# NCAR/SPERR

Measured on AMD Instinct MI355X. Metric: compress+decompress GB/s/GPU on 256^3 fp32 chunks @ BPP=2.0; bitstream-exact vs ref, higher is better.
Workload: dtype f64; 1 GPU; synthetic 1024^3 fp32 turbulence per GPU, 256^3 chunks, BPP=2.0, step = compress + decompress, volume and container resident in HBM; chunks_per_gpu=64, parallelism=chunks farmed over 1 GPU(s), no collective

## Files before the change

sperr_amd/csrc/engine.hip:

```cpp
#include <algorithm>
#include <array>
#include <chrono>
#include <cstdlib>
#include <cstring>
#include <atomic>
#include <deque>
#include <map>
#include <memory>
#include <condition_variable>
#include <mutex>
#include <numeric>
#include <thread>
#include <string>
#include <vector>

#include "../../include/sperr_hip.h"
#include "engine_internal.h"
#include "host_container.hpp"
#include "speck_dec.h"
#include "speck_enc.h"
#include "speck_tree_host.hpp"
#include "outlier.h"
#include "xform.h"

// ... 1094 lines not shown
  e.pixCntStride = (size_t)kMaxPlanes * 2 * P.nPixTiles;
  TAKE(e.pixCnt, uint32_t, e.pixCntStride * B);
  TAKE(e.pixOff, uint32_t, e.pixCntStride * B);
  e.streamStride = streamWords;
  TAKE(e.stream, uint64_t, streamWords * B);
#undef TAKE
  return true;
}

size_t enc_bytes_for(const ShapePlan& P, uint32_t B, uint64_t raw_budget, bool alias = true)
{
  Arena probe;
  probe.base = reinterpret_cast<char*>(uintptr_t(4096));
  probe.cap = ~size_t(0) / 2;
  EncBatchBufs tmp;
  carve_enc(probe, P, std::max<uint32_t>(B, 1), raw_budget, tmp, alias);
  return probe.used;
}
size_t enc_bytes_per_chunk(const ShapePlan& P, uint64_t raw_budget, bool alias = true)
{
  return enc_bytes_for(P, 1, raw_budget, alias);
}

int reset_enc_pass(hipStream_t st, const EncBatchBufs& bb, uint32_t B)
{
  const EncBuffers& e = bb.eb;
  HIP_CHECK(hipMemsetAsync(e.bplane, 0xff, e.pixStride * B, st));
  HIP_CHECK(hipMemsetAsync(e.M, 0xff, e.nodeStride * B, st));
  HIP_CHECK(hipMemsetAsync(e.mask, 0, std::max<size_t>(e.maskStride, 1) * B * sizeof(uint64_t), st));
  HIP_CHECK(hipMemsetAsync(e.stream, 0, e.streamStride * B * sizeof(uint64_t), st));
  return 0;
}

bool fuse_xy(const ShapePlan& P)
{
  if (P.fwd.size() < 2 || P.fwd[0].axis != 0 || P.fwd[1].axis != 1)
    return false;
  for (int a = 0; a < 3; a++)
    if (P.fwd[0].region[a] != P.dims[a] || P.fwd[1].region[a] != P.dims[a])
      return false;
  return lift_xy_applicable(P.dims);
}

bool fuse_xyz(const ShapePlan& P)
{
  if (!fuse_xy(P) || P.fwd.size() < 3 || P.fwd[2].axis != 2)
    return false;
  for (int a = 0; a < 3; a++)
    if (P.fwd[2].region[a] != P.dims[a])
      return false;
  return lift_xyz_applicable(P.dims);
}

int pass_fuse(const ShapePlan& P, size_t k, uint32_t inner[3])
{
  const LiftPass& ps = P.fwd[k];
  inner[0] = inner[1] = inner[2] = 0;
  for (size_t j = k + 1; j < P.fwd.size(); j++)
    for (int a = 0; a < 3; a++)
      inner[a] = std::max(inner[a], P.fwd[j].region[a]);
  bool nested = k + 1 >= P.fwd.size();
  for (size_t j = k + 1; j < P.fwd.size(); j++)
    nested = nested || (P.fwd[j].region[0] == inner[0] && P.fwd[j].region[1] == inner[1] &&
                        P.fwd[j].region[2] == inner[2]);
  if (!nested)
    return -1;
  bool covers = true;
  for (int a = 0; a < 3; a++)
    covers = covers && inner[a] >= ps.region[a];
  return covers ? 0 : 1;
}

bool plan_fusable(const ShapePlan& P)
{
  if (P.fwd.empty())
    return false;
  uint32_t inner[3];
  for (size_t k = 0; k < P.fwd.size(); k++)
    if (pass_fuse(P, k, inner) < 0)
      return false;
  if (fuse_xy(P) && (pass_fuse(P, 0, inner) != 0 || pass_fuse(P, 1, inner) != 0))
    return false;
  return true;
}

template <typename T>
int float_stages(hipStream_t ss, const ShapePlan& P, EncBatchBufs& bb, uint32_t nb, const uint32_t cd[3],
                 const T* d_src, VolDesc vd, bool orgAligned, bool wantRange)
{
  EncBuffers& e = bb.eb;
  const bool fuse = !P.fwd.empty();
  const int io = std::is_same<T, float>::value ? 1 : 2;
  if (launch_condition<T>(ss, d_src, vd, bb.geom, nb, cd, P.nstrides, bb.strideMean, bb.strideMeanStride,
                          bb.vals, bb.valsStride, e.cst, !fuse, wantRange, orgAligned))
    return -1;
  size_t k0 = 0;
  const bool fuseMax = plan_fusable(P);
  if (fuse_xyz(P)) {
    LiftFuse lf;
    if (fuseMax && pass_fuse(P, 2, lf.inner) > 0)
      lf.mode = 1;
    if (launch_lift_xyz(ss, true, bb.vals, bb.valsStride, nb, cd, e.cst, io, const_cast<T*>(d_src), vd,
                        bb.geom, &lf))
      return -1;
    k0 = 3;
  }
  else if (fuse_xy(P)) {
    if (launch_lift_xy(ss, true, bb.vals, bb.valsStride, nb, cd, e.cst, io, const_cast<T*>(d_src), vd,
                       bb.geom))
      return -1;
    k0 = 2;
  }
  for (size_t k = k0; k < P.fwd.size(); k++) {
    const LiftPass& ps = P.fwd[k];
    LiftFuse lf;
    if (fuseMax && pass_fuse(P, k, lf.inner) > 0)
      lf.mode = 1;
    if (launch_lift(ss, true, bb.vals, bb.valsStride, nb, cd, ps.axis, ps.region, e.cst, k == 0 ? io : 0,
                    const_cast<T*>(d_src), vd, bb.geom, &lf))
      return -1;
  }
  return 0;
}

int unalias_coder(hipStream_t ss, Engine& E, const ShapePlan& P, EncBatchBufs& bb, uint32_t nb)
{
  HIP_CHECK(hipStreamSynchronize(ss));
  if (E.wideScratch.ensure(bb.coderBytes + 4096))
    return -1;
  Arena W;
  W.base = static_cast<char*>(E.wideScratch.p);
  W.cap = E.wideScratch.n;
  if (!carve_enc_coder(W, nullptr, P, nb, bb.eb))
    return -1;
  bb.aliased = false;
  return 0;
}

template <typename T>
int wide_retry_prepare(hipStream_t ss, Engine& E, const ShapePlan& P, EncBatchBufs& bb, uint32_t nb,
                       const uint32_t cd[3], const T* d_src, VolDesc vd, bool orgAligned, bool wantRange)
{
  if (unalias_coder(ss, E, P, bb, nb))
    return -1;
  g_dbg_counter[0]++;
  return float_stages<T>(ss, P, bb, nb, cd, d_src, vd, orgAligned, wantRange);
}

int psnr_q_search(hipStream_t st, const ShapePlan& P, EncBatchBufs& bb, uint32_t nb, double psnr,
                  std::vector<CoderState>& hc, std::vector<CoderState>& got)
{
  EncBuffers& e = bb.eb;
  hc.assign(nb, CoderState{});
  HIP_CHECK(hipMemcpyAsync(hc.data(), e.cst, nb * sizeof(CoderState), hipMemcpyDeviceToHost, st));
  HIP_CHECK(hipStreamSynchronize(st));
  std::vector<double> tmse(nb, 0.0);
  bool any = false;
  for (uint32_t i = 0; i < nb; i++) {
// ... 1748 lines not shown
    double* boxVals = nullptr;
    size_t boxStride = 0;
    ChunkGeom* d_bricks = nullptr;
    if (fbrick) {
      for (size_t k = 3; k < P.fwd.size(); k++)
        for (int a = 0; a < 3; a++)
          bbox[a] = std::max(bbox[a], P.fwd[k].region[a]);
      boxStride = round_up((size_t)bbox[0] * bbox[1] * bbox[2], 64);
      const size_t geomOff = round_up((size_t)nb * boxStride * 8, 256);
      if (E.decBox[q].ensure(geomOff + (size_t)nb * sizeof(ChunkGeom) + 256))
        return -1;
      boxVals = static_cast<double*>(E.decBox[q].p);
      d_bricks = reinterpret_cast<ChunkGeom*>(static_cast<char*>(E.decBox[q].p) + geomOff);
      S.bricks.resize(nb);
      for (uint32_t i = 0; i < nb; i++) {
        S.bricks[i].org[0] = (uint32_t)((size_t)i * bb.valsStride);
        S.bricks[i].org[1] = S.bricks[i].org[2] = 0;
      }
      HIP_CHECK(hipMemcpyAsync(d_bricks, S.bricks.data(), nb * sizeof(ChunkGeom), hipMemcpyHostToDevice, ss));
    }
    const size_t perLevel = slice ? 2 : 3;
    auto sub_volume = [&](size_t k) -> int {
      if (!mr || !mr->nlev)
        return 0;
      const size_t h = mr->nlev - (k / perLevel + 1);
      const auto& r = mr->cres[h];
      const uint32_t blocks = capped_blocks((r[0] * r[1] * r[2] + kThreads - 1) / kThreads, nb);
      LAUNCH_K(k_sub_volume, dim3(blocks, nb), dim3(kThreads), 0, ss, bb.vals, bb.valsStride, d.cst, bb.geom,
               cd[0], cd[1], cd[0], cd[1], cd[2], r[0], r[1], r[2], mr->grid[0], mr->grid[1], mr->d_level[h]);
      return 0;
    };
    auto dequant_fuse = [&](size_t k, LiftFuse& lf) {
      if (b.fuseDq && pass_fuse(P, k, lf.inner) > 0) {
        lf.mode = 2;
        lf.coef = bb.coef32;
        lf.coefStride = d.coefStride;
        lf.sign = d.sign;
        lf.signStride = d.signStride;
        lf.sigNew = d.sigNew;
        lf.sigOld = d.sigOld;
        lf.maskStride = d.maskPixStride;
        lf.dst = d.st;
        lf.coefSigned = d.refPlanes ? 1 : 0;
      }
      if (b.compactElems) {
        lf.bufx = b.cbox[0];
        lf.bufy = b.cbox[1];
      }
      if (fbrick) {
        lf.bufx = bbox[0];
        lf.bufy = bbox[1];
      }
    };
    for (size_t k = P.fwd.size(); k-- > ((fxyz || fbrick) ? 3u : fxy ? 2u : 0u);) {
      const LiftPass& ps = P.fwd[k];
      if (k % perLevel == perLevel - 1 && sub_volume(k))
        return -1;
      LiftFuse lf;
      dequant_fuse(k, lf);
      const bool last = k == 0 && !S.outliers;
      if (launch_lift(ss, false, fbrick ? boxVals : bb.vals, fbrick ? boxStride : bb.valsStride, nb, cd, ps.axis,
                      ps.region, d.cst, last ? io : 0, d_dst, vd, bb.geom, &lf, last ? bb.crop : nullptr))
        return -1;
    }
    if (fbrick) {
      LiftFuse lf;
      dequant_fuse(2, lf);
      lf.noMean = 1;
      const VolDesc brickVol{{cd[0], cd[1], cd[2]}};
      if (launch_lift_xyz(ss, false, boxVals, boxStride, nb, cd, d.cst, 2, bb.vals, brickVol, d_bricks, &lf))
        return -1;
    }
    if (fxyz) {
      if (sub_volume(2))
        return -1;
      LiftFuse lf;
      dequant_fuse(2, lf);
      if (launch_lift_xyz(ss, false, bb.vals, bb.valsStride, nb, cd, d.cst, io, d_dst, vd, bb.geom, &lf, bb.crop))
        return -1;
    }
    if (fxy && slice && sub_volume(1))
      return -1;
    if (fxy && launch_lift_xy(ss, false, bb.vals, bb.valsStride, nb, cd, d.cst, io, d_dst, vd, bb.geom, bb.crop))
      return -1;
    if (S.outliers) {
      HIP_CHECK(hipStreamWaitEvent(ss, E.evOutl[q], 0));
      if (launch_outlier_apply(ss, S.ob, d.cst, bb.vals, bb.valsStride))
        return -1;
      HIP_CHECK(hipMemcpyAsync(S.hoc.data(), S.ob.oc, nb * sizeof(OutlierChunk), hipMemcpyDeviceToHost, ss));
      HIP_CHECK(hipStreamSynchronize(ss));
      for (auto& o : S.hoc)
        if (o.error) {
          fprintf(stderr, "[sperr_hip] outlier decoder failed (code %u)\n", o.error);
          return -1;
        }
    }
    if ((P.fwd.empty() || S.outliers) &&
        launch_scatter<T>(ss, d_dst, vd, bb.geom, nb, cd, bb.vals, bb.valsStride, d.cst, bb.crop))
      return -1;
    return 0;
  }
  int collect_states(const Batch& b)
  {
    for (uint32_t q = 0; q < b.nsub; q++) {
      SubHost& S = (*b.subs)[q];
      if (S.nb == 0)
        continue;
      hipStream_t ss = b.nsub > 1 ? E.sub[q] : st;
      if (S.bb.db.lisStamps && q == 0) {
        g_lis_stamps_host.assign(64, 0);
        const uint32_t sc = getenv("SPERR_HIP_STAMP_CHUNK")
                                ? std::min<uint32_t>(S.nb - 1, (uint32_t)atoi(getenv("SPERR_HIP_STAMP_CHUNK")))
                                : 0u;
        HIP_CHECK(hipMemcpyAsync(g_lis_stamps_host.data(), S.bb.db.lisStamps + (size_t)sc * 64, 64 * 8,
                                 hipMemcpyDeviceToHost, ss));
// ... 1348 lines not shown
```

sperr_amd/csrc/xform.h:

```cpp
#ifndef SPERR_AMD_XFORM_H
#define SPERR_AMD_XFORM_H

#include <string.h>

#include "common.h"

namespace sperrhip {

struct LiftConsts {
  double alpha, beta, gamma, delta, eps, inv_eps;
};
LiftConsts lift_consts();

template <typename T>
int launch_condition(hipStream_t stream, const T* vol, VolDesc vd, const ChunkGeom* geom,
                     uint32_t nchunks, const uint32_t cdims[3], uint32_t nstrides,
                     double* strideMean, size_t strideMeanStride, double* vals,
                     size_t valsStride, CoderState* st, bool gather, bool want_range = false,
                     bool org_x_aligned = false);

template <typename T>
int launch_scatter(hipStream_t stream, T* vol, VolDesc vd, const ChunkGeom* geom,
                   uint32_t nchunks, const uint32_t cdims[3], const double* vals,
                   size_t valsStride, const CoderState* st, const CropGeom* crop = nullptr);

struct DecState;
struct LiftFuse {
  int mode = 0;
  uint32_t inner[3] = {0, 0, 0};
  const uint32_t* coef = nullptr;
  size_t coefStride = 0;
  const uint64_t* sign = nullptr;
  size_t signStride = 0;
  const uint64_t* sigNew = nullptr;
  const uint64_t* sigOld = nullptr;
  size_t maskStride = 0;
  const DecState* dst = nullptr;
  int coefSigned = 0;
  int noMean = 0;
  uint32_t bufx = 0, bufy = 0;
};

int launch_lift(hipStream_t stream, bool forward, double* vals, size_t valsStride,
                uint32_t nchunks, const uint32_t cdims[3], int axis, const uint32_t region[3],
                CoderState* st, int io = 0, void* volume = nullptr, VolDesc vd = VolDesc{},
                const ChunkGeom* geom = nullptr, const LiftFuse* fuse = nullptr,
                const CropGeom* crop = nullptr);

bool lift_xy_applicable(const uint32_t cdims[3]);
int launch_lift_xy(hipStream_t stream, bool forward, double* vals, size_t valsStride,
                   uint32_t nchunks, const uint32_t cdims[3], const CoderState* st, int io,
                   void* volume, VolDesc vd, const ChunkGeom* geom, const CropGeom* crop = nullptr);

bool lift_xyz_applicable(const uint32_t cdims[3]);
int launch_lift_xyz(hipStream_t stream, bool forward, double* vals, size_t valsStride, uint32_t nchunks,
                    const uint32_t cdims[3], CoderState* st, int io, void* volume, VolDesc vd,
                    const ChunkGeom* geom, const LiftFuse* fuse, const CropGeom* crop = nullptr);

int launch_maxabs_q(hipStream_t stream, const double* vals, size_t valsStride, uint32_t nchunks,
                    uint32_t n, CoderState* st, bool have_max = false);
int launch_make_q_wide(hipStream_t stream, uint32_t nchunks, CoderState* st);
int launch_mark_wide(hipStream_t stream, uint32_t nchunks, CoderState* st);

int launch_mse(hipStream_t stream, const double* vals, size_t valsStride, uint32_t nchunks,
               uint32_t n, double* partial, size_t partialStride, CoderState* st);

__host__ __device__ inline unsigned long long order_key(double v)
{
  unsigned long long b;
  memcpy(&b, &v, 8);
  return (b >> 63) ? ~b : (b | 0x8000000000000000ull);
}
__host__ __device__ inline double order_key_value(unsigned long long k)
{
  const unsigned long long b = (k >> 63) ? (k & 0x7fffffffffffffffull) : ~k;
  double v;
  memcpy(&v, &b, 8);
  return v;
}

int launch_quantize(hipStream_t stream, bool wide, const double* vals, size_t valsStride,
                    uint32_t nchunks, uint32_t n, void* coef, size_t coefStride, uint64_t* sign,
                    size_t signStride, int8_t* msb, size_t msbStride, const CoderState* st);

int launch_inv_quantize(hipStream_t stream, bool wide, const void* coef, size_t coefStride,
                        const uint64_t* sign, size_t signStride, uint32_t nchunks, uint32_t n,
                        double* vals, size_t valsStride, const CoderState* st,
                        const uint64_t* sigNew = nullptr, const uint64_t* sigOld = nullptr,
                        size_t maskStride = 0, const DecState* dst = nullptr);

}

#endif
```

sperr_amd/csrc/xform.hip:

```cpp
#include <type_traits>

#include "xform.h"
#include "speck_dec.h"

namespace sperrhip {


constexpr int kSumStrides = 64, kSumSeg = 64;


template <typename T>
__global__ void __launch_bounds__(kThreads)
k_stride_sums(const T* __restrict__ vol, VolDesc vd, const ChunkGeom* geom, uint32_t cx,
              uint32_t cy, uint32_t cz, uint32_t nstrides, uint32_t ssz, double* strideMean,
              size_t strideMeanStride, CoderState* st, int want_range)
{
  __shared__ double tile[kSumStrides][kSumSeg + 1];
  __shared__ uint32_t sh_differs;
  double vmax = -INFINITY, vnegmax = -INFINITY;
  const uint32_t c = blockIdx.y;
  const uint32_t s0 = blockIdx.x * kSumStrides;
  const ChunkGeom g = geom[c];
  const size_t vx = vd.dims[0], vy = vd.dims[1];
  const T first = vol[((size_t)g.org[2] * vy + g.org[1]) * vx + g.org[0]];
// ... 736 lines not shown
                                           uint32_t jhi, uint32_t tid, const LiftConsts& K)
{
  const uint32_t nseg = (cx + kSeg - 1) / kSeg;
  const uint32_t ntask = (jhi - jlo) * nseg;
#pragma unroll 1
  for (uint32_t t = tid; t < ntask; t += NT) {
    const uint32_t rows = jhi - jlo, sg = t / rows, rb = jlo + (t - sg * rows);
    const double* row = src + (size_t)rb * RS + sg * kSeg;
    double r[16];
#pragma unroll
    for (int k = 0; k < 16; k++)
      r[k] = row[k];
    lift16<FORWARD>(r, K);
    double* out = dst + (size_t)rb * RS + 4 + sg * kSeg;
#pragma unroll
    for (int k = 0; k < kSeg; k++)
      if (sg * kSeg + k < cx)
        out[k] = r[4 + k];
  }
}

template <bool FORWARD, bool APRON, int NT>
__device__ __forceinline__ void xyz_lift_y(const double* src, double* dst, uint32_t RS, uint32_t cx, uint32_t nt,
                                           uint32_t tid, const LiftConsts& K)
{
  const uint32_t nq = (nt + kSeg - 1) / kSeg;
  const uint32_t ntask = nq * cx;
#pragma unroll 1
  for (uint32_t t = tid; t < ntask; t += NT) {
    const uint32_t q = t / cx, x = t - q * cx;
    const double* top = src + (size_t)(q * kSeg) * RS + 4 + x;
    double r[16];
#pragma unroll
    for (int k = 0; k < 16; k++)
      r[k] = top[(size_t)k * RS];
    lift16<FORWARD>(r, K);
#pragma unroll
    for (int k = 0; k < kSeg; k++) {
      if (q * kSeg + k < nt) {
        double* row = dst + (size_t)(4 + q * kSeg + k) * RS;
        if (APRON)
          xyz_put(row, x, cx, r[4 + k]);
        else
          row[4 + x] = r[4 + k];
      }
    }
  }
}

template <int IO>
__global__ void __launch_bounds__(kXYZThreadsF) __attribute__((amdgpu_waves_per_eu(kXYZThreadsF / 256, kXYZThreadsF / 256)))
k_lift_xyz_fwd(double* vals, size_t valsStride, uint32_t cx, uint32_t cy, uint32_t cz, LiftConsts K,
               CoderState* st, const void* volume, VolDesc vd, const ChunkGeom* geom, int wantMax,
               uint32_t in0, uint32_t in1, uint32_t in2, uint32_t nseg)
{
  static_assert(IO == 1 || IO == 2, "float or double volume");
  using VT = typename std::conditional<IO == 1, float, double>::type;
  const uint32_t c = blockIdx.y;
  if (st[c].is_const != 0)
    return;
  const uint32_t tid = threadIdx.x;
  const uint32_t seg = blockIdx.x % nseg, npairsAll = (cz + 1) / 2;
  const uint32_t mA = seg == 0 ? 0u : (uint32_t)((uint64_t)npairsAll * seg / nseg);
  const uint32_t mB = seg + 1 == nseg ? npairsAll : (uint32_t)((uint64_t)npairsAll * (seg + 1) / nseg);
  const uint32_t zFirst = mA >= 6 ? 2 * (mA - 6) : 0u;
  const uint32_t zEnd = seg + 1 == nseg ? cz : 2 * mB - 1;
  const uint32_t y0 = (blockIdx.x / nseg) * kXYZRows;
  const uint32_t nt = min((uint32_t)kXYZRows, cy - y0);
  const uint32_t RS = xyz_row_stride(cx);
  double* sm = reinterpret_cast<double*>(dyn_smem);
  const uint32_t bufN = (uint32_t)kXYZStaged * RS;
  const uint32_t xe = cx - cx / 2, ye = cy - cy / 2, ze = cz - cz / 2;
  const VT* vol = reinterpret_cast<const VT*>(volume);
  const size_t vsy = vd.dims[0], vsz = (size_t)vd.dims[0] * vd.dims[1];
  const VT* volc = vol + ((size_t)geom[c].org[2] * vsz + (size_t)geom[c].org[1] * vsy + geom[c].org[0]);
  double* buf = vals + c * valsStride;
  const size_t sliceN = (size_t)cx * cy;
  const double mean = st[c].mean;

  const uint32_t nstage = (uint32_t)kXYZStaged * cx;
  uint32_t pk[kXYZStageF];
#pragma unroll
  for (int k = 0; k < kXYZStageF; k++) {
    const uint32_t q = tid + (uint32_t)k * kXYZThreadsF;
    const uint32_t j = q / cx, x = q - j * cx;
    pk[k] = (j << 27) | (reflect_index((int)y0 - kXYHalo + (int)j, (int)cy) << 12) | x;
  }
  const uint32_t npos = nt * cx;
  uint32_t srow[kXYZPosF], ooff[kXYZPosF];
  uint32_t outerMask = 0;
#pragma unroll
  for (int k = 0; k < kXYZPosF; k++) {
    const uint32_t q = tid + (uint32_t)k * kXYZThreadsF;
    const uint32_t row = q / cx, col = q - row * cx, y = y0 + row;
    srow[k] = ((row + kXYHalo) << 16) | col;
    const uint32_t drow = (y & 1) ? ye + (y >> 1) : (y >> 1), dcol = (col & 1) ? xe + (col >> 1) : (col >> 1);
    ooff[k] = drow * cx + dcol;
    if (!(dcol < in0 && drow < in1))
      outerMask |= 1u << k;
  }
  double sxe[kXYZPosF], sxo[kXYZPosF], d1p[kXYZPosF], e1p[kXYZPosF], d2p[kXYZPosF];
#pragma unroll
  for (int k = 0; k < kXYZPosF; k++)
    sxe[k] = sxo[k] = d1p[k] = e1p[k] = d2p[k] = 0.0;
  double vmax = 0.0;
  auto emit = [&](int k, uint32_t zp, double v) {
    buf[(size_t)zp * sliceN + ooff[k]] = v;
    if (wantMax && (((outerMask >> k) & 1u) || zp >= in2))
      vmax = fmax(vmax, fabs(v));
  };

  VT pre[kXYZStageF];
  auto issue = [&](uint32_t z) {
    const VT* src = volc + (size_t)z * vsz;
#pragma unroll
    for (int k = 0; k < kXYZStageF; k++)
      pre[k] = (tid + (uint32_t)k * kXYZThreadsF) < nstage
                   ? src[(size_t)((pk[k] >> 12) & 0x7fffu) * vsy + (pk[k] & 0xfffu)] : (VT)0;
  };
  issue(zFirst);
  for (uint32_t z = zFirst; z < zEnd; z++) {
    uint32_t RSv = RS, tidv = tid;
    asm volatile("" : "+s"(RSv), "+v"(tidv));
#pragma unroll
    for (int k = 0; k < kXYZStageF; k++)
      asm volatile("" : "+v"(pk[k]));
#pragma unroll
    for (int k = 0; k < kXYZPosF; k++)
      asm volatile("" : "+v"(srow[k]), "+v"(ooff[k]));
    double* A = sm + ((z & 1) ? bufN : 0u);
    double* B = sm + ((z & 1) ? 0u : bufN);
#pragma unroll
    for (int k = 0; k < kXYZStageF; k++)
      if ((tid + (uint32_t)k * kXYZThreadsF) < nstage)
        xyz_put(A + (pk[k] >> 27) * RSv, pk[k] & 0xfffu, cx, (double)pre[k] - mean);
    if (z + 1 < zEnd)
      issue(z + 1);
    XYZ_LDS_BARRIER();
    xyz_lift_x<true, kXYZThreadsF>(A, B, RSv, cx, 0, kXYZStaged, tidv, K);
    XYZ_LDS_BARRIER();
    xyz_lift_y<true, false, kXYZThreadsF>(B, A, RSv, cx, nt, tidv, K);
    XYZ_LDS_BARRIER();
    const uint32_t m = z >> 1;
    if (z & 1) {
#pragma unroll
      for (int k = 0; k < kXYZPosF; k++)
        if ((tid + (uint32_t)k * kXYZThreadsF) < npos)
          sxo[k] = A[(srow[k] >> 16) * RSv + 4 + (srow[k] & 0xffffu)];
    }
    else {
#pragma unroll
      for (int k = 0; k < kXYZPosF; k++) {
        if ((tid + (uint32_t)k * kXYZThreadsF) >= npos)
          continue;
        const double v = A[(srow[k] >> 16) * RSv + 4 + (srow[k] & 0xffffu)];
        if (m >= 1) {
          const double d1n = fma(K.alpha, sxe[k] + v, sxo[k]);
          const double e1n = fma(K.beta, (m == 1 ? d1n : d1p[k]) + d1n, sxe[k]);
          if (m >= 2) {
            const double d2n = fma(K.gamma, e1p[k] + e1n, d1p[k]);
            const double e2 = K.eps * fma(K.delta, (m == 2 ? d2n : d2p[k]) + d2n, e1p[k]);
// ... 29 lines not shown
    }
    else {
      const uint32_t M = cz / 2;
      const double e1M = fma(K.beta, d1p[k] + d1p[k], sxe[k]);
      const double d2a = fma(K.gamma, e1p[k] + e1M, d1p[k]);
      const double e2a = K.eps * fma(K.delta, d2p[k] + d2a, e1p[k]);
      const double e2L = K.eps * fma(K.delta, d2a + d2a, e1M);
      emit(k, M - 1, e2a);
      emit(k, ze + M - 1, (-K.inv_eps) * d2a);
      emit(k, M, e2L);
    }
  }
  if (wantMax) {
    for (int d = 32; d > 0; d >>= 1)
      vmax = fmax(vmax, __shfl_xor(vmax, d, 64));
    if ((tid & 63) == 0 && vmax > 0.0)
      atomicMax(reinterpret_cast<unsigned long long*>(&st[c].maxabs),
                (unsigned long long)__double_as_longlong(vmax));
  }
}

template <int IO, bool SG, bool kCrop = false>
__global__ void __launch_bounds__(kXYZThreadsI) __attribute__((amdgpu_waves_per_eu(kXYZThreadsI / 256, kXYZThreadsI / 256)))
k_lift_xyz_inv(const double* vals, size_t valsStride, uint32_t cx, uint32_t cy, uint32_t cz, LiftConsts K,
               const CoderState* st, void* volume, VolDesc vd, const GeomOf<kCrop>* geom, LiftFuse F, uint32_t nseg)
{
  static_assert(IO == 1 || IO == 2, "float or double volume");
  using VT = typename std::conditional<IO == 1, float, double>::type;
  const uint32_t c = blockIdx.y;
  const uint32_t tid = threadIdx.x;
  const uint32_t seg = blockIdx.x % nseg, npairsAll = cz / 2;
  const uint32_t mA = seg == 0 ? 0u : (uint32_t)((uint64_t)npairsAll * seg / nseg);
  const uint32_t mB = seg + 1 == nseg ? npairsAll : (uint32_t)((uint64_t)npairsAll * (seg + 1) / nseg);
  const uint32_t mFirst = mA >= 6 ? mA - 6 : 0u;
  const uint32_t y0 = (blockIdx.x / nseg) * kXYZRows;
  const uint32_t nt = min((uint32_t)kXYZRows, cy - y0);
  const uint32_t RS = xyz_row_stride(cx);
  double* sm = reinterpret_cast<double*>(dyn_smem);
  const uint32_t bufN = (uint32_t)kXYZStaged * RS;
  const uint32_t xe = cx - cx / 2, ye = cy - cy / 2, ze = cz - cz / 2;
  VT* vol = reinterpret_cast<VT*>(volume);
  const size_t vsy = vd.dims[0], vsz = (size_t)vd.dims[0] * vd.dims[1];
  VT* volc = vol;
  CropGeom cg{};
  uint32_t wy0 = 0, wy1 = 0;
  if constexpr (kCrop) {
    cg = geom[c];
    wy0 = max(y0, cg.lo[1]) - y0;
    wy1 = min(y0 + nt, cg.hi[1]);
    if (y0 + wy0 >= wy1)
      return;
    wy1 -= y0;
  }
  else
    volc = vol + ((size_t)geom[c].org[2] * vsz + (size_t)geom[c].org[1] * vsy + geom[c].org[0]);
  auto crop_row = [&](uint32_t z, uint32_t r) -> VT* { return vol + crop_addr(cg, vd, cg.lo[0], y0 + r, z); };
  (void)crop_row;
  const double* buf = vals + c * valsStride;
  const size_t sliceN = (size_t)cx * cy;
  const uint32_t bufx = F.bufx ? F.bufx : cx;
  const size_t bufSlice = (size_t)bufx * (F.bufy ? F.bufy : cy);
  const double mean = st[c].mean;
  const uint32_t lane = tid & 63u, wave = tid >> 6, nwaves = kXYZThreadsI / 64;

  if (st[c].is_const != 0) {
    if constexpr (kCrop) {
      const uint32_t w = cg.hi[0] - cg.lo[0], nr = wy1 - wy0;
      for (uint32_t z = cg.lo[2] + seg; z < cg.hi[2]; z += nseg)
        for (uint32_t k = tid; k < nr * w; k += kXYZThreadsI)
          crop_row(z, wy0 + k / w)[k % w] = (VT)mean;
    }
    else
    for (uint32_t z = seg; z < cz; z += nseg)
      for (uint32_t k = tid; k < nt * cx; k += kXYZThreadsI)
        volc[(size_t)z * vsz + (size_t)(y0 + k / cx) * vsy + k % cx] = (VT)mean;
    return;
  }

  const uint32_t npos = (uint32_t)kXYZStaged * cx;
  uint32_t pk[kXYZPosI];
  uint32_t innerMask = 0;
#pragma unroll
  for (int k = 0; k < kXYZPosI; k++) {
    const uint32_t q = tid + (uint32_t)k * kXYZThreadsI;
    const uint32_t j = q / cx, x = q - j * cx, y = reflect_index((int)y0 - kXYHalo + (int)j, (int)cy);
    const uint32_t drow = (y & 1) ? ye + (y >> 1) : (y >> 1), dcol = (x & 1) ? xe + (x >> 1) : (x >> 1);
    pk[k] = (j << 27) | (y << 12) | x;
    if (dcol < F.inner[0] && drow < F.inner[1])
      innerMask |= 1u << k;
  }
  const bool dequant = F.mode == 2 && !st[c].wide;
  const double fq = dequant ? st[c].q : 0.0;
  const uint32_t* coef = F.coef + c * F.coefStride;
  const uint64_t* sign = F.sign + c * F.signStride;
  const bool haveMasks = dequant && F.sigNew != nullptr && F.dst != nullptr;
  const uint64_t* mNew = haveMasks ? F.sigNew + c * F.maskStride : sign;
  const uint64_t* mOld = haveMasks ? F.sigOld + c * F.maskStride : sign;
  const uint32_t lastPl = haveMasks ? (uint32_t)F.dst[c].lastPlane : 0u;
  const uint32_t initNew = haveMasks ? (1u << lastPl) + (1u << lastPl) - (1u << lastPl) / 2 - 1 : 0u;
  const uint32_t initOld = (haveMasks && lastPl < 31) ? (2u << lastPl) + (2u << lastPl) - (2u << lastPl) / 2 - 1 : 0u;
  const int scheme = (SG && dequant && F.dst) ? coef_scheme(F.dst[c]) : 0;
  const bool two = scheme == 2;
  auto sg_value = [&](uint32_t sv) -> double {
    double d = fq * (double)coef_scheme_mag(sv, two);
    return __hiloint2double(__double2hiint(d) ^ (int)(sv & 0x80000000u), __double2loint(d));
  };
  auto fetch = [&](int k, uint32_t zp) -> double {
    const uint32_t y = (pk[k] >> 12) & 0x7fffu, x = pk[k] & 0xfffu;
    const uint32_t drow = (y & 1) ? ye + (y >> 1) : (y >> 1), dcol = (x & 1) ? xe + (x >> 1) : (x >> 1);
    const size_t idx = (size_t)zp * sliceN + drow * cx + dcol;
    const bool inBox = ((innerMask >> k) & 1u) && zp < F.inner[2];
    if (!dequant && !inBox && F.bufx)
      return 0.0;
    if (dequant && !inBox) {
      if (SG && scheme)
        return sg_value(coef[idx]);
      uint32_t v = coef[idx];
      const uint32_t sh = (uint32_t)(idx & 63);
      const uint64_t sgw = sign[idx >> 6], mnw = mNew[idx >> 6], mow = mOld[idx >> 6];
      const uint32_t fill = ((mnw >> sh) & 1ull) ? initNew : (((mow >> sh) & 1ull) ? initOld : 0u);
      v = v ? v : fill;
      return fq * (double)v * (((sgw >> sh) & 1ull) ? 1.0 : -1.0);
    }
    return buf[(size_t)zp * bufSlice + drow * bufx + dcol];
  };
  uint32_t flip = 0;
  auto stage = [&](int k, double v) {
    uint32_t p = pk[k];
    asm volatile("" : "+v"(p));
    (sm + (flip ? bufN : 0u))[(p >> 27) * RS + 4 + (p & 0xfffu)] = v;
  };
  auto stage_all = [&](const double (&v)[kXYZPosI]) {
#pragma unroll
    for (int k = 0; k < kXYZPosI; k++)
      if ((tid + (uint32_t)k * kXYZThreadsI) < npos)
        stage(k, v[k]);
  };
  auto store_rows = [&](uint32_t z, uint32_t which) {
    const double* X = sm + (which ? bufN : 0u);
    if constexpr (kCrop) {
      if (z - cg.lo[2] >= cg.hi[2] - cg.lo[2])
        return;
      for (uint32_t r = wy0 + wave; r < wy1; r += nwaves) {
        VT* dstrow = crop_row(z, r);
        const double* srow = X + (size_t)(kXYHalo + r) * RS + 4;
        for (uint32_t x = cg.lo[0] + lane; x < cg.hi[0]; x += 64)
          dstrow[x - cg.lo[0]] = (VT)(F.noMean ? srow[x] : srow[x] + mean);
      }
      return;
    }
    for (uint32_t r = wave; r < nt; r += nwaves) {
      VT* dstrow = volc + (size_t)z * vsz + (size_t)(y0 + r) * vsy;
      const double* srow = X + (size_t)(kXYHalo + r) * RS + 4;
      if (F.noMean) {
        for (uint32_t x = lane; x < cx; x += 64)
          dstrow[x] = (VT)srow[x];
      }
      else
        for (uint32_t x = lane; x < cx; x += 64)
          dstrow[x] = (VT)(srow[x] + mean);
    }
  };
  auto finish_slice = [&](uint32_t z) {
// ... 37 lines not shown
  const uint32_t* mNew32 = reinterpret_cast<const uint32_t*>(mNew);
  const uint32_t* mOld32 = reinterpret_cast<const uint32_t*>(mOld);
  uint32_t activeMask = 0;
#pragma unroll
  for (int k = 0; k < kXYZPosI; k++)
    if ((tid + (uint32_t)k * kXYZThreadsI) < npos)
      activeMask |= 1u << k;
    else
      pk[k] = pk[0];
  uint32_t boxAny = 0;
#pragma unroll
  for (int k = 0; k < kXYZPosI; k++)
    boxAny |= __ballot((innerMask >> k) & 1u) != 0ull ? 1u << k : 0u;
  boxAny = (uint32_t)__builtin_amdgcn_readfirstlane((int)boxAny);
  auto pos_off = [&](int k, uint32_t& drow, uint32_t& dcol) {
    const uint32_t y = (pk[k] >> 12) & 0x7fffu, x = pk[k] & 0xfffu;
    drow = (y & 1) ? ye + (y >> 1) : (y >> 1);
    dcol = (x & 1) ? xe + (x >> 1) : (x >> 1);
  };
  const bool fastLoads = dequant && F.inner[2] <= ze && (!SG || scheme != 0);
  uint32_t boxLds = 0, boxSlot0 = 0;
  uint32_t* boxRows = reinterpret_cast<uint32_t*>(sm + 2 * (size_t)bufN) + (size_t)nwaves * (kXYZPosI * 2 * 64);
  if (SG && fastLoads) {
    uint32_t reg = 0;
#pragma unroll
    for (int k = 0; k < kXYZPosI; k++) {
      const uint64_t inb = __ballot((innerMask >> k) & 1u), act = __ballot((activeMask >> k) & 1u);
      if (inb == 0x5555555555555555ull && act == ~0ull && (cx & 63u) == 0)
        reg |= 1u << k;
    }
    reg = (uint32_t)__builtin_amdgcn_readfirstlane((int)reg);
    uint32_t* cnt = reinterpret_cast<uint32_t*>(sm);
    if (lane == 0)
      cnt[wave] = (uint32_t)__popc(reg);
    XYZ_LDS_BARRIER();
    uint32_t before = 0, total = 0;
    for (uint32_t w = 0; w < nwaves; w++) {
      const uint32_t v = cnt[w];
      before += w < wave ? v : 0u;
      total += v;
    }
    XYZ_LDS_BARRIER();
    if (total <= (uint32_t)kXYZBoxSlots && reg == (1u << kXYZPosI) - 1u) {
      boxLds = reg;
      boxSlot0 = before;
    }
  }
  uint32_t* myBox = boxRows + (size_t)boxSlot0 * 64;
  auto pre_issue = [&](uint32_t m) {
#pragma unroll
    for (int k = 0; k < kXYZPosI; k++) {
      uint32_t drow, dcol;
      pos_off(k, drow, dcol);
      const uint32_t off = drow * cx + dcol;
      __builtin_amdgcn_global_load_lds(coef + ((size_t)m * sliceN + off), myPre + (k * 2) * 64, 4, 0, 0);
      __builtin_amdgcn_global_load_lds(coef + ((size_t)(ze + m) * sliceN + off), myPre + (k * 2 + 1) * 64, 4, 0, 0);
    }
    if (SG && boxLds != 0 && m < F.inner[2]) {
#pragma unroll
      for (int k = 0; k < kXYZPosI; k++) {
        uint32_t drow, dcol;
        pos_off(k, drow, dcol);
        const uint32_t x0h = ((pk[k] & 0xfffu) - lane) >> 1;
        const uint32_t* src = reinterpret_cast<const uint32_t*>(buf + ((size_t)m * bufSlice + (size_t)drow * bufx + x0h)) + lane;
        __builtin_amdgcn_global_load_lds(src, myBox + k * 64, 4, 0, 0);
      }
    }
  };
  if (fastLoads && mFirst < mB)
    pre_issue(mFirst);
#endif
  for (uint32_t m = mFirst; m < mB; m++) {
    const bool mine = m >= mA;
#pragma unroll
    for (int k = 0; k < kXYZPosI; k++)
      asm volatile("" : "+v"(pk[k]));
#if XYZ_INV_PREFETCH == 2
    if (SG && fastLoads) {
      asm volatile("s_waitcnt vmcnt(0)" ::: "memory");
      const bool boxWave = boxAny != 0 && m < F.inner[2];
      if (boxWave && boxLds != 0) {
#pragma unroll
        for (int k = 0; k < kXYZPosI; k++) {
          const double lo = sg_value(myPre[(k * 2) * 64 + lane]);
          const double hi = sg_value(myPre[(k * 2 + 1) * 64 + lane]);
          const double bxv = reinterpret_cast<const double*>(myBox + k * 64)[lane >> 1];
          zstep(k, m, mine, true, (lane & 1u) ? lo : bxv, hi);
        }
      }
      else {
#pragma unroll
      for (int g = 0; g < kXYZPosI; g += kXYZGroupI) {
        __builtin_amdgcn_sched_barrier(0);
        double bx[kXYZGroupI];
        uint32_t boxm = 0;
        if (boxWave) {
#pragma unroll
          for (int kk = 0; kk < kXYZGroupI; kk++) {
            const int k = g + kk;
            if (k >= kXYZPosI)
              continue;
            uint32_t drow, dcol;
            pos_off(k, drow, dcol);
            const bool inBox = ((innerMask >> k) & 1u) != 0;
            boxm |= inBox ? 1u << kk : 0u;
            bx[kk] = buf[inBox ? (size_t)m * bufSlice + drow * bufx + dcol : (size_t)0];
          }
        }
#pragma unroll
        for (int kk = 0; kk < kXYZGroupI; kk++) {
          const int k = g + kk;
          if (k >= kXYZPosI)
            continue;
          const double lo = sg_value(myPre[(k * 2) * 64 + lane]);
          const double hi = sg_value(myPre[(k * 2 + 1) * 64 + lane]);
          zstep(k, m, mine, ((activeMask >> k) & 1u) != 0, ((boxm >> kk) & 1u) ? bx[kk] : lo, hi);
        }
      }
      }
      __builtin_amdgcn_sched_barrier(0);
      if (m + 1 < mB)
        pre_issue(m + 1);
      __builtin_amdgcn_sched_barrier(0);
    }
    else if (!SG && fastLoads) {
      asm volatile("s_waitcnt vmcnt(0)" ::: "memory");
#pragma unroll
      for (int g = 0; g < kXYZPosI; g += kXYZGroupI) {
        __builtin_amdgcn_sched_barrier(0);
        constexpr int NV = 2 * kXYZGroupI;
        uint32_t sgw[NV], mnw[NV], mow[NV], cv[NV], shv[NV], boxm = 0;
        double bx[kXYZGroupI];
#pragma unroll
        for (int j = 0; j < NV; j++) {
          const int k = g + j / 2;
          if (k >= kXYZPosI)
            continue;
          const uint32_t zp = (j & 1) ? ze + m : m;
          uint32_t drow, dcol;
          pos_off(k, drow, dcol);
          const size_t idx = (size_t)zp * sliceN + drow * cx + dcol;
          sgw[j] = sign32[idx >> 5];
          mnw[j] = mNew32[idx >> 5];
          mow[j] = mOld32[idx >> 5];
          if ((j & 1) == 0) {
            const bool inBox = ((innerMask >> k) & 1u) && zp < F.inner[2];
            boxm |= inBox ? 1u << j : 0u;
            bx[j / 2] = buf[inBox ? (size_t)zp * bufSlice + drow * bufx + dcol : (size_t)0];
          }
          cv[j] = myPre[(k * 2 + (j & 1)) * 64 + lane];
          shv[j] = (uint32_t)idx & 31u;
        }
        double val[NV];
#pragma unroll
        for (int j = 0; j < NV; j++) {
          if (g + j / 2 >= kXYZPosI)
            continue;
          const uint32_t fill = ((mnw[j] >> shv[j]) & 1u) ? initNew : (((mow[j] >> shv[j]) & 1u) ? initOld : 0u);
          const uint32_t v = cv[j] ? cv[j] : fill;
          const double dq = fq * (double)v * (((sgw[j] >> shv[j]) & 1u) ? 1.0 : -1.0);
          val[j] = ((j & 1) == 0 && ((boxm >> j) & 1u)) ? bx[j / 2] : dq;
        }
#pragma unroll
        for (int kk = 0; kk < kXYZGroupI; kk++)
          if (g + kk < kXYZPosI)
            zstep(g + kk, m, mine, ((activeMask >> (g + kk)) & 1u) != 0, val[2 * kk], val[2 * kk + 1]);
      }
      __builtin_amdgcn_sched_barrier(0);
      if (m + 1 < mB)
        pre_issue(m + 1);
      __builtin_amdgcn_sched_barrier(0);
    }
    else
#endif
    {
#pragma unroll
      for (int k = 0; k < kXYZPosI; k++) {
        if ((k % 3) == 0)
          __builtin_amdgcn_sched_barrier(0);
        if ((tid + (uint32_t)k * kXYZThreadsI) >= npos)
          continue;
        const double E = fetch(k, m), O = fetch(k, ze + m);
        zstep(k, m, mine, true, E, O);
      }
    }
    if (m >= 2 && mine)
      finish_slice(2 * m - 3);
    if (m >= 1 && mine) {
      stage_all(e2p);
      finish_slice(2 * m - 2);
    }
  }
  if (seg + 1 != nseg)
    return;
// ... 400 lines not shown
                          reinterpret_cast<const void*>(&k_lift_xy<true, 2>),
                          reinterpret_cast<const void*>(&k_lift_xy<false, 1>),
                          reinterpret_cast<const void*>(&k_lift_xy<false, 2>),
                          reinterpret_cast<const void*>(&k_lift_xy<false, 1, true>),
                          reinterpret_cast<const void*>(&k_lift_xy<false, 2, true>)};
    for (const void* f : fns)
      if (set_max_dyn_lds(f, 160 * 1024))
        return -1;
  }
  const int R = xy_rows(cdims[0], cdims[1]);
  if (R <= 0 || (io != 1 && io != 2))
    return -1;
  const size_t smem = (size_t)(R + 2 * kXYHalo) * (cdims[0] + 1) * sizeof(double);
  const uint32_t ntile = (cdims[1] + R - 1) / R;
  const dim3 grid(ntile * cdims[2], nchunks);
  const LiftConsts K = lift_consts();
#define XY_ARGS vals, valsStride, cdims[0], cdims[1], cdims[2], R, K, st, volume, vd, geom
  if (forward) {
    if (io == 1)
      LAUNCH_K((k_lift_xy<true, 1>), grid, dim3(kXYThreads), smem, stream, XY_ARGS);
    else
      LAUNCH_K((k_lift_xy<true, 2>), grid, dim3(kXYThreads), smem, stream, XY_ARGS);
  }
  else if (crop) {
#define CROP_ARGS vals, valsStride, cdims[0], cdims[1], cdims[2], R, K, st, volume, vd, crop
    if (io == 1)
      LAUNCH_K((k_lift_xy<false, 1, true>), grid, dim3(kXYThreads), smem, stream, CROP_ARGS);
    else
      LAUNCH_K((k_lift_xy<false, 2, true>), grid, dim3(kXYThreads), smem, stream, CROP_ARGS);
#undef CROP_ARGS
  }
  else {
    if (io == 1)
      LAUNCH_K((k_lift_xy<false, 1>), grid, dim3(kXYThreads), smem, stream, XY_ARGS);
    else
      LAUNCH_K((k_lift_xy<false, 2>), grid, dim3(kXYThreads), smem, stream, XY_ARGS);
  }
#undef XY_ARGS
  HIP_CHECK(hipGetLastError());
  return 0;
}

bool lift_xyz_applicable(const uint32_t cdims[3])
{
  if (cdims[0] < 9 || cdims[1] < 9 || cdims[2] < 9)
    return false;
  return (size_t)kXYZStaged * cdims[0] <= (size_t)kXYZPosI * kXYZThreadsI &&
         (size_t)kXYZStaged * cdims[0] <= (size_t)kXYZStageF * kXYZThreadsF &&
         (size_t)kXYZRows * cdims[0] <= (size_t)kXYZPosF * kXYZThreadsF && cdims[0] < 4096 && cdims[1] < 32768;
}

int launch_lift_xyz(hipStream_t stream, bool forward, double* vals, size_t valsStride, uint32_t nchunks,
                    const uint32_t cdims[3], CoderState* st, int io, void* volume, VolDesc vd,
                    const ChunkGeom* geom, const LiftFuse* fuse, const CropGeom* crop)
{
  if (!lift_xyz_applicable(cdims) || (io != 1 && io != 2) || (crop && forward))
    return -1;
  const LiftFuse F = fuse ? *fuse : LiftFuse{};
  size_t smem = 2 * (size_t)kXYZStaged * xyz_row_stride(cdims[0]) * sizeof(double);
#if XYZ_INV_PREFETCH == 2
  if (!forward)
    smem += (size_t)kXYZThreadsI * kXYZPosI * 2 * sizeof(uint32_t) +
            (size_t)kXYZBoxSlots * 64 * sizeof(uint32_t);
#endif
  {
    const void* fns[10] = {reinterpret_cast<const void*>(&k_lift_xyz_fwd<1>), reinterpret_cast<const void*>(&k_lift_xyz_fwd<2>),
                           reinterpret_cast<const void*>(&k_lift_xyz_inv<1, false>), reinterpret_cast<const void*>(&k_lift_xyz_inv<2, false>),
                           reinterpret_cast<const void*>(&k_lift_xyz_inv<1, true>), reinterpret_cast<const void*>(&k_lift_xyz_inv<2, true>),
                           reinterpret_cast<const void*>(&k_lift_xyz_inv<1, false, true>), reinterpret_cast<const void*>(&k_lift_xyz_inv<2, false, true>),
                           reinterpret_cast<const void*>(&k_lift_xyz_inv<1, true, true>), reinterpret_cast<const void*>(&k_lift_xyz_inv<2, true, true>)};
    for (const void* f : fns)
      if (set_max_dyn_lds(f, 160 * 1024))
        return -1;
  }
  const uint32_t ntile = (cdims[1] + kXYZRows - 1) / kXYZRows;
  uint32_t nseg = 1;
  while (nseg < 4 && (size_t)ntile * nchunks * nseg < 512 && cdims[2] / (2 * nseg) >= 24)
    nseg *= 2;
  const dim3 grid(ntile * nseg, nchunks);
  const LiftConsts K = lift_consts();
  if (forward) {
    const int wantMax = F.mode == 1 ? 1 : 0;
    if (io == 1)
      LAUNCH_K((k_lift_xyz_fwd<1>), grid, dim3(kXYZThreadsF), smem, stream, vals, valsStride, cdims[0], cdims[1],
               cdims[2], K, st, volume, vd, geom, wantMax, F.inner[0], F.inner[1], F.inner[2], nseg);
    else
      LAUNCH_K((k_lift_xyz_fwd<2>), grid, dim3(kXYZThreadsF), smem, stream, vals, valsStride, cdims[0], cdims[1],
               cdims[2], K, st, volume, vd, geom, wantMax, F.inner[0], F.inner[1], F.inner[2], nseg);
  }
  else {
    const bool sg = F.mode == 2 && F.coefSigned != 0;
#define XYZ_INV_LAUNCH(io_, sg_)                                                                                    \
  LAUNCH_K((k_lift_xyz_inv<io_, sg_>), grid, dim3(kXYZThreadsI), smem, stream, vals, valsStride, cdims[0], cdims[1], \
           cdims[2], K, st, volume, vd, geom, F, nseg)
#define XYZ_CROP_LAUNCH(io_, sg_)                                                                                   \
  LAUNCH_K((k_lift_xyz_inv<io_, sg_, true>), grid, dim3(kXYZThreadsI), smem, stream, vals, valsStride, cdims[0],      \
           cdims[1], cdims[2], K, st, volume, vd, crop, F, nseg)
    if (crop) {
      if (io == 1 && sg)
        XYZ_CROP_LAUNCH(1, true);
      else if (io == 1)
        XYZ_CROP_LAUNCH(1, false);
      else if (sg)
        XYZ_CROP_LAUNCH(2, true);
      else
        XYZ_CROP_LAUNCH(2, false);
    }
    else if (io == 1) {
      if (sg)
        XYZ_INV_LAUNCH(1, true);
      else
        XYZ_INV_LAUNCH(1, false);
    }
    else {
      if (sg)
        XYZ_INV_LAUNCH(2, true);
      else
        XYZ_INV_LAUNCH(2, false);
    }
#undef XYZ_INV_LAUNCH
#undef XYZ_CROP_LAUNCH
  }
  HIP_CHECK(hipGetLastError());
  return 0;
}

template <typename T>
int launch_condition(hipStream_t stream, const T* vol, VolDesc vd, const ChunkGeom* geom,
                     uint32_t nchunks, const uint32_t cdims[3], uint32_t nstrides,
                     double* strideMean, size_t strideMeanStride, double* vals,
                     size_t valsStride, CoderState* st, bool gather, bool want_range,
                     bool org_x_aligned)
{
  const uint32_t n = cdims[0] * cdims[1] * cdims[2];
  const uint32_t ssz = n / nstrides;
  const uint32_t perLoad = 8 * (16 / (uint32_t)sizeof(T));
  const bool rowsPath = cdims[0] % perLoad == 0 && ssz % cdims[0] == 0 &&
                        vd.dims[0] % (16 / sizeof(T)) == 0 &&
                        reinterpret_cast<uintptr_t>(vol) % 16 == 0 && org_x_aligned;
  if (rowsPath)
    LAUNCH_K(k_stride_sums_rows<T>, dim3((nstrides + 63) / 64, nchunks), dim3(64), 0, stream, vol,
// ... 130 lines not shown
```

Before: 63.90 GB/s.

## Extend fused xyz lifting kernel across multiple wavelet levels via compact box buffers

Forward and inverse transforms now apply the fused 3-axis lifting kernel to every coarser level whose three passes share a region, instead of only the first level followed by per-axis lift launches. The forward kernel writes the low-pass box into a compact ping-pong scratch buffer (aliased onto the coef32 area), which the next level reads as its input volume. The inverse path does the same through vals and the decoder's lis buffer. This removes several per-axis passes over memory per level. In exchange it adds indexing complexity and aliasing of scratch buffers, and it falls back to one level when the buffers are too small.

```diff
diff --git a/sperr_amd/csrc/engine.hip b/sperr_amd/csrc/engine.hip
--- a/sperr_amd/csrc/engine.hip
+++ b/sperr_amd/csrc/engine.hip
@@ -1170,6 +1170,40 @@
   return lift_xyz_applicable(P.dims);
 }
 
+bool level_xyz(const ShapePlan& P, size_t l)
+{
+  if (P.fwd.size() < 3 * l + 3)
+    return false;
+  for (int a = 0; a < 3; a++) {
+    if (P.fwd[3 * l + a].axis != a)
+      return false;
+    for (int d = 0; d < 3; d++)
+      if (P.fwd[3 * l + a].region[d] != P.fwd[3 * l].region[d])
+        return false;
+  }
+  return lift_xyz_applicable(P.fwd[3 * l].region);
+}
+
+size_t fused_levels(const ShapePlan& P)
+{
+  static const bool perAxis = getenv("SPERR_HIP_LEVELS_PER_AXIS") && atoi(getenv("SPERR_HIP_LEVELS_PER_AXIS")) != 0;
+  if (!fuse_xyz(P))
+    return 0;
+  size_t n = 1;
+  while (!perAxis && level_xyz(P, n))
+    n++;
+  return n;
+}
+
+void level_box_elems(const ShapePlan& P, size_t nlev, size_t elems[2])
+{
+  elems[0] = elems[1] = 0;
+  for (size_t l = 1; l < nlev; l++) {
+    const uint32_t* r = P.fwd[3 * l].region;
+    elems[(l - 1) & 1] = std::max(elems[(l - 1) & 1], (size_t)r[0] * r[1] * r[2]);
+  }
+}
+
 int pass_fuse(const ShapePlan& P, size_t k, uint32_t inner[3])
 {
   const LiftPass& ps = P.fwd[k];
@@ -1215,13 +1249,40 @@
   size_t k0 = 0;
   const bool fuseMax = plan_fusable(P);
   if (fuse_xyz(P)) {
-    LiftFuse lf;
-    if (fuseMax && pass_fuse(P, 2, lf.inner) > 0)
-      lf.mode = 1;
-    if (launch_lift_xyz(ss, true, bb.vals, bb.valsStride, nb, cd, e.cst, io, const_cast<T*>(d_src), vd,
-                        bb.geom, &lf))
-      return -1;
-    k0 = 3;
+    size_t nlev = fuseMax ? fused_levels(P) : 1;
+    size_t belems[2];
+    level_box_elems(P, nlev, belems);
+    const size_t boxOff1 = round_up(belems[0], 32);
+    if ((boxOff1 + belems[1]) * sizeof(double) > e.coefStride * sizeof(uint32_t))
+      nlev = 1;
+    double* const boxBase = reinterpret_cast<double*>(bb.coef32);
+    const size_t boxStride = e.coefStride / 2;
+    for (size_t l = 0; l < nlev; l++) {
+      const uint32_t* r = P.fwd[3 * l].region;
+      LiftFuse lf;
+      const int pf = pass_fuse(P, 3 * l + 2, lf.inner);
+      if (fuseMax && pf > 0)
+        lf.mode = 1;
+      XyzLevel lv;
+      if (l + 1 < nlev)
+        lv.box = boxBase + ((l & 1) ? boxOff1 : 0);
+      lv.boxStride = boxStride;
+      if (l == 0) {
+        if (launch_lift_xyz(ss, true, bb.vals, bb.valsStride, nb, cd, e.cst, io, const_cast<T*>(d_src), vd,
+                            bb.geom, &lf, nullptr, &lv))
+          return -1;
+        continue;
+      }
+      lv.pitchx = cd[0];
+      lv.pitchy = cd[1];
+      lv.volStride = boxStride;
+      lv.noMean = 1;
+      const VolDesc boxVol{{r[0], r[1], r[2]}};
+      if (launch_lift_xyz(ss, true, bb.vals, bb.valsStride, nb, r, e.cst, 2, boxBase + (((l - 1) & 1) ? boxOff1 : 0),
+                          boxVol, bb.geom, &lf, nullptr, &lv))
+        return -1;
+    }
+    k0 = 3 * nlev;
   }
   else if (fuse_xy(P)) {
     if (launch_lift_xy(ss, true, bb.vals, bb.valsStride, nb, cd, e.cst, io, const_cast<T*>(d_src), vd,
@@ -3076,15 +3137,52 @@
         lf.bufy = bbox[1];
       }
     };
-    for (size_t k = P.fwd.size(); k-- > ((fxyz || fbrick) ? 3u : fxy ? 2u : 0u);) {
+    size_t nlev = 1;
+    double* lvBuf[2] = {bb.vals, reinterpret_cast<double*>(d.lis[0])};
+    const size_t lvStride[2] = {bb.valsStride, d.lisStride};
+    if (fxyz && b.compactElems && b.fuseDq && S.maxWide == 0) {
+      nlev = fused_levels(P);
+      size_t belems[2];
+      level_box_elems(P, std::min(nlev + 1, (P.fwd.size() + 2) / 3), belems);
+      if (belems[0] > lvStride[0] || belems[1] > lvStride[1])
+        nlev = 1;
+    }
+    double* axVals = fbrick ? boxVals : bb.vals;
+    size_t axStride = fbrick ? boxStride : bb.valsStride;
+    if (nlev > 1) {
+      axVals = lvBuf[(nlev - 1) & 1];
+      axStride = lvStride[(nlev - 1) & 1];
+    }
+    for (size_t k = P.fwd.size(); k-- > (nlev > 1 ? 3u * nlev : (fxyz || fbrick) ? 3u : fxy ? 2u : 0u);) {
       const LiftPass& ps = P.fwd[k];
       if (k % perLevel == perLevel - 1 && sub_volume(k))
         return -1;
       LiftFuse lf;
       dequant_fuse(k, lf);
+      if (nlev > 1) {
+        lf.bufx = P.fwd[3 * nlev].region[0];
+        lf.bufy = P.fwd[3 * nlev].region[1];
+      }
       const bool last = k == 0 && !S.outliers;
-      if (launch_lift(ss, false, fbrick ? boxVals : bb.vals, fbrick ? boxStride : bb.valsStride, nb, cd, ps.axis,
+      if (launch_lift(ss, false, axVals, axStride, nb, cd, ps.axis,
                       ps.region, d.cst, last ? io : 0, d_dst, vd, bb.geom, &lf, last ? bb.crop : nullptr))
+        return -1;
+    }
+    for (size_t l = nlev; l-- > 1;) {
+      const uint32_t* r = P.fwd[3 * l].region;
+      LiftFuse lf;
+      dequant_fuse(3 * l + 2, lf);
+      if (lf.mode != 2)
+        return -1;
+      lf.bufx = lf.inner[0];
+      lf.bufy = lf.inner[1];
+      lf.coefx = cd[0];
+      lf.coefy = cd[1];
+      lf.noMean = 1;
+      lf.volStride = lvStride[(l - 1) & 1];
+      const VolDesc boxVol{{r[0], r[1], r[2]}};
+      if (launch_lift_xyz(ss, false, lvBuf[l & 1], lvStride[l & 1], nb, r, d.cst, 2, lvBuf[(l - 1) & 1], boxVol, bb.geom,
+                          &lf))
         return -1;
     }
     if (fbrick) {
diff --git a/sperr_amd/csrc/xform.h b/sperr_amd/csrc/xform.h
--- a/sperr_amd/csrc/xform.h
+++ b/sperr_amd/csrc/xform.h
@@ -39,6 +39,16 @@
   int coefSigned = 0;
   int noMean = 0;
   uint32_t bufx = 0, bufy = 0;
+  uint32_t coefx = 0, coefy = 0;
+  size_t volStride = 0;
+};
+
+struct XyzLevel {
+  uint32_t pitchx = 0, pitchy = 0;
+  size_t volStride = 0;
+  int noMean = 0;
+  double* box = nullptr;
+  size_t boxStride = 0;
 };
 
 int launch_lift(hipStream_t stream, bool forward, double* vals, size_t valsStride,
@@ -55,7 +65,8 @@
 bool lift_xyz_applicable(const uint32_t cdims[3]);
 int launch_lift_xyz(hipStream_t stream, bool forward, double* vals, size_t valsStride, uint32_t nchunks,
                     const uint32_t cdims[3], CoderState* st, int io, void* volume, VolDesc vd,
-                    const ChunkGeom* geom, const LiftFuse* fuse, const CropGeom* crop = nullptr);
+                    const ChunkGeom* geom, const LiftFuse* fuse, const CropGeom* crop = nullptr,
+                    const XyzLevel* level = nullptr);
 
 int launch_maxabs_q(hipStream_t stream, const double* vals, size_t valsStride, uint32_t nchunks,
                     uint32_t n, CoderState* st, bool have_max = false);
diff --git a/sperr_amd/csrc/xform.hip b/sperr_amd/csrc/xform.hip
--- a/sperr_amd/csrc/xform.hip
+++ b/sperr_amd/csrc/xform.hip
@@ -812,7 +812,7 @@
 __global__ void __launch_bounds__(kXYZThreadsF) __attribute__((amdgpu_waves_per_eu(kXYZThreadsF / 256, kXYZThreadsF / 256)))
 k_lift_xyz_fwd(double* vals, size_t valsStride, uint32_t cx, uint32_t cy, uint32_t cz, LiftConsts K,
                CoderState* st, const void* volume, VolDesc vd, const ChunkGeom* geom, int wantMax,
-               uint32_t in0, uint32_t in1, uint32_t in2, uint32_t nseg)
+               uint32_t in0, uint32_t in1, uint32_t in2, uint32_t nseg, XyzLevel L)
 {
   static_assert(IO == 1 || IO == 2, "float or double volume");
   using VT = typename std::conditional<IO == 1, float, double>::type;
@@ -833,10 +833,13 @@
   const uint32_t xe = cx - cx / 2, ye = cy - cy / 2, ze = cz - cz / 2;
   const VT* vol = reinterpret_cast<const VT*>(volume);
   const size_t vsy = vd.dims[0], vsz = (size_t)vd.dims[0] * vd.dims[1];
-  const VT* volc = vol + ((size_t)geom[c].org[2] * vsz + (size_t)geom[c].org[1] * vsy + geom[c].org[0]);
+  const VT* volc = L.volStride ? vol + (size_t)c * L.volStride
+                               : vol + ((size_t)geom[c].org[2] * vsz + (size_t)geom[c].org[1] * vsy + geom[c].org[0]);
   double* buf = vals + c * valsStride;
-  const size_t sliceN = (size_t)cx * cy;
-  const double mean = st[c].mean;
+  const uint32_t opx = L.pitchx ? L.pitchx : cx;
+  const size_t sliceN = (size_t)opx * (L.pitchy ? L.pitchy : cy);
+  double* boxc = L.box ? L.box + (size_t)c * L.boxStride : nullptr;
+  const double mean = L.noMean ? 0.0 : st[c].mean;
 
   const uint32_t nstage = (uint32_t)kXYZStaged * cx;
   uint32_t pk[kXYZStageF];
@@ -855,7 +858,7 @@
     const uint32_t row = q / cx, col = q - row * cx, y = y0 + row;
     srow[k] = ((row + kXYHalo) << 16) | col;
     const uint32_t drow = (y & 1) ? ye + (y >> 1) : (y >> 1), dcol = (col & 1) ? xe + (col >> 1) : (col >> 1);
-    ooff[k] = drow * cx + dcol;
+    ooff[k] = drow * opx + dcol;
     if (!(dcol < in0 && drow < in1))
       outerMask |= 1u << k;
   }
@@ -865,8 +868,14 @@
     sxe[k] = sxo[k] = d1p[k] = e1p[k] = d2p[k] = 0.0;
   double vmax = 0.0;
   auto emit = [&](int k, uint32_t zp, double v) {
-    buf[(size_t)zp * sliceN + ooff[k]] = v;
-    if (wantMax && (((outerMask >> k) & 1u) || zp >= in2))
+    const bool outer = ((outerMask >> k) & 1u) || zp >= in2;
+    double* dst = buf + ((size_t)zp * sliceN + ooff[k]);
+    if (boxc && !outer) {
+      const uint32_t drow = (y0 + (srow[k] >> 16) - kXYHalo) >> 1, dcol = (srow[k] & 0xffffu) >> 1;
+      dst = boxc + ((size_t)zp * in1 + drow) * in0 + dcol;
+    }
+    *dst = v;
+    if (wantMax && outer)
       vmax = fmax(vmax, fabs(v));
   };
 
@@ -1002,12 +1011,15 @@
       return;
     wy1 -= y0;
   }
+  else if (F.volStride)
+    volc = vol + (size_t)c * F.volStride;
   else
     volc = vol + ((size_t)geom[c].org[2] * vsz + (size_t)geom[c].org[1] * vsy + geom[c].org[0]);
   auto crop_row = [&](uint32_t z, uint32_t r) -> VT* { return vol + crop_addr(cg, vd, cg.lo[0], y0 + r, z); };
   (void)crop_row;
   const double* buf = vals + c * valsStride;
-  const size_t sliceN = (size_t)cx * cy;
+  const uint32_t cpx = F.coefx ? F.coefx : cx;
+  const size_t sliceN = (size_t)cpx * (F.coefy ? F.coefy : cy);
   const uint32_t bufx = F.bufx ? F.bufx : cx;
   const size_t bufSlice = (size_t)bufx * (F.bufy ? F.bufy : cy);
   const double mean = st[c].mean;
@@ -1058,7 +1070,7 @@
   auto fetch = [&](int k, uint32_t zp) -> double {
     const uint32_t y = (pk[k] >> 12) & 0x7fffu, x = pk[k] & 0xfffu;
     const uint32_t drow = (y & 1) ? ye + (y >> 1) : (y >> 1), dcol = (x & 1) ? xe + (x >> 1) : (x >> 1);
-    const size_t idx = (size_t)zp * sliceN + drow * cx + dcol;
+    const size_t idx = (size_t)zp * sliceN + drow * cpx + dcol;
     const bool inBox = ((innerMask >> k) & 1u) && zp < F.inner[2];
     if (!dequant && !inBox && F.bufx)
       return 0.0;
@@ -1202,7 +1214,7 @@
     for (int k = 0; k < kXYZPosI; k++) {
       uint32_t drow, dcol;
       pos_off(k, drow, dcol);
-      const uint32_t off = drow * cx + dcol;
+      const uint32_t off = drow * cpx + dcol;
       __builtin_amdgcn_global_load_lds(coef + ((size_t)m * sliceN + off), myPre + (k * 2) * 64, 4, 0, 0);
       __builtin_amdgcn_global_load_lds(coef + ((size_t)(ze + m) * sliceN + off), myPre + (k * 2 + 1) * 64, 4, 0, 0);
     }
@@ -1289,7 +1301,7 @@
           const uint32_t zp = (j & 1) ? ze + m : m;
           uint32_t drow, dcol;
           pos_off(k, drow, dcol);
-          const size_t idx = (size_t)zp * sliceN + drow * cx + dcol;
+          const size_t idx = (size_t)zp * sliceN + drow * cpx + dcol;
           sgw[j] = sign32[idx >> 5];
           mnw[j] = mNew32[idx >> 5];
           mow[j] = mOld32[idx >> 5];
@@ -1796,11 +1808,15 @@
 
 int launch_lift_xyz(hipStream_t stream, bool forward, double* vals, size_t valsStride, uint32_t nchunks,
                     const uint32_t cdims[3], CoderState* st, int io, void* volume, VolDesc vd,
-                    const ChunkGeom* geom, const LiftFuse* fuse, const CropGeom* crop)
-{
-  if (!lift_xyz_applicable(cdims) || (io != 1 && io != 2) || (crop && forward))
+                    const ChunkGeom* geom, const LiftFuse* fuse, const CropGeom* crop, const XyzLevel* level)
+{
+  if (!lift_xyz_applicable(cdims) || (io != 1 && io != 2) || (crop && forward) || (level && !forward))
     return -1;
   const LiftFuse F = fuse ? *fuse : LiftFuse{};
+  const XyzLevel L = level ? *level : XyzLevel{};
+  if (L.box && (F.inner[0] > cdims[0] - cdims[0] / 2 || F.inner[1] > cdims[1] - cdims[1] / 2 ||
+                F.inner[2] > cdims[2] - cdims[2] / 2))
+    return -1;
   size_t smem = 2 * (size_t)kXYZStaged * xyz_row_stride(cdims[0]) * sizeof(double);
 #if XYZ_INV_PREFETCH == 2
   if (!forward)
@@ -1827,10 +1843,10 @@
     const int wantMax = F.mode == 1 ? 1 : 0;
     if (io == 1)
       LAUNCH_K((k_lift_xyz_fwd<1>), grid, dim3(kXYZThreadsF), smem, stream, vals, valsStride, cdims[0], cdims[1],
-               cdims[2], K, st, volume, vd, geom, wantMax, F.inner[0], F.inner[1], F.inner[2], nseg);
+               cdims[2], K, st, volume, vd, geom, wantMax, F.inner[0], F.inner[1], F.inner[2], nseg, L);
     else
       LAUNCH_K((k_lift_xyz_fwd<2>), grid, dim3(kXYZThreadsF), smem, stream, vals, valsStride, cdims[0], cdims[1],
-               cdims[2], K, st, volume, vd, geom, wantMax, F.inner[0], F.inner[1], F.inner[2], nseg);
+               cdims[2], K, st, volume, vd, geom, wantMax, F.inner[0], F.inner[1], F.inner[2], nseg, L);
   }
   else {
     const bool sg = F.mode == 2 && F.coefSigned != 0;
```

After: 63.94 GB/s (median of 2 runs). Within noise of the previous version (+0.1%).
